# gengyuchao/SonicScribe

Measured on AMD Instinct MI355X. Metric: 20s-segments/sec/node + RTF, GLM-ASR-Nano bf16, batch=32, 1/2/4/8 MI355X, higher is better.
Workload: dtype bf16

## Files before the change

### sonicscribe_amd/csrc/attn.hip

```cpp
#include "common.h"
#include "kernels.h"
#include "int8_util.h"
#include <type_traits>


typedef unsigned u32x2_t __attribute__((ext_vector_type(2)));
__device__ __forceinline__ float rows_sum(float v) {
    u32x2_t a = __builtin_amdgcn_permlane16_swap(__float_as_uint(v), __float_as_uint(v), false, false);
    const float s = __uint_as_float(a[0]) + __uint_as_float(a[1]);
    u32x2_t b = __builtin_amdgcn_permlane32_swap(__float_as_uint(s), __float_as_uint(s), false, false);
    return __uint_as_float(b[0]) + __uint_as_float(b[1]);
}
__device__ __forceinline__ float rows_max(float v) {
    u32x2_t a = __builtin_amdgcn_permlane16_swap(__float_as_uint(v), __float_as_uint(v), false, false);
    const float s = fmaxf(__uint_as_float(a[0]), __uint_as_float(a[1]));
    u32x2_t b = __builtin_amdgcn_permlane32_swap(__float_as_uint(s), __float_as_uint(s), false, false);
    return fmaxf(__uint_as_float(b[0]), __uint_as_float(b[1]));
}

template <int HD> __device__ __forceinline__ int kswz(int row) {
    if (HD == 64) return ((row >> 1) & 1) | (((row >> 3) & 3) << 1);
    return ((row & 3) | (((row >> 3) & 1) << 2)) << 1;
}

// ... 274 lines not shown
    int n;
    if (a.P) {
        const int N = (a.Hq + 2 * a.Hkv) * HD;
        const int w = tid, vi = w / HALF, i = w % HALF;
        const bool act = w < (G + 2) * HALF;
        float x1 = 0.f, x2 = 0.f;
        if (act) {
            const int col = (vi < G ? (kvh * G + vi) : vi == G ? (a.Hq + kvh) : (a.Hq + a.Hkv + kvh)) * HD + i;
            if (a.dq.sca) {
                x1 = deq1(a.dq, a.P, a.ksplit, a.mpad, b, col, N); x2 = deq1(a.dq, a.P, a.ksplit, a.mpad, b, col + HALF, N);
            } else {
                float v1[8], v2[8];
#pragma unroll
                for (int ks = 0; ks < 8; ++ks) {
                    const float* p = a.P + ((long)(ks < a.ksplit ? ks : 0) * a.mpad + b) * N + col;
                    v1[ks] = p[0]; v2[ks] = p[HALF];
                }
#pragma unroll
                for (int ks = 0; ks < 8; ++ks)
                    if (ks < a.ksplit) { x1 += v1[ks]; x2 += v2[ks]; }
            }
        }
        n = min(max(a.kv_len[b], 1), a.ctx_max);
        if (act) {
            const int pos = n - 1;
            x1 = rT<T>(x1); x2 = rT<T>(x2);
            float o1 = x1, o2 = x2;
            if (vi <= G) {
                const float c = a.cs[(long)pos * HD + i], sn = a.cs[(long)pos * HD + HALF + i];
                o1 = rT<T>(rT<T>(x1 * c) + rT<T>(-x2 * sn));
                o2 = rT<T>(rT<T>(x2 * c) + rT<T>(x1 * sn));
            }
            const int row = vi < G ? vi : (vi == G ? GMAX : GMAX + 1);
            const T b1 = (T)o1, b2 = (T)o2;
            s_q[row][i] = b1; s_q[row][HALF + i] = b2;
            if (vi == G) { Kc[(long)pos * HD + i] = b1; Kc[(long)pos * HD + HALF + i] = b2; }
            if (vi == G + 1) { Vc[(long)pos * HD + i] = b1; Vc[(long)pos * HD + HALF + i] = b2; }
        }
        __syncthreads();
    } else {
        n = min(max(a.kv_len[b], 1), a.ctx_max);
    }
    KT(a, 1);
    V8 qf[4];
#pragma unroll
    for (int hs = 0; hs < 4; ++hs) {
        const V8 t = a.P ? *(const V8*)&s_q[r < G ? r : 0][hs * 32 + g * 8]
                         : *(const V8*)((const T*)a.Q + (long)b * a.Hq * HD + (kvh * G + (r < G ? r : 0)) * HD + hs * 32 + g * 8);
#pragma unroll
        for (int j = 0; j < 8; ++j) qf[hs][j] = r < G ? t[j] : (T)0.f;
    }
    float m[GMAX], lsum = 0.f, acc[GMAX][8];
#pragma unroll
    for (int h = 0; h < GMAX; ++h) {
        m[h] = -1e30f;
#pragma unroll
        for (int i = 0; i < 8; ++i) acc[h][i] = 0.f;
    }
    auto step = [&](int k0, const V8 (&kd)[4], const V8 (&vd)[4], int limit) {
        f32x4 st = {0.f, 0.f, 0.f, 0.f};
#pragma unroll
        for (int hs = 0; hs < 4; ++hs) st = ET<T>::mfma(kd[hs], qf[hs], st);
        float sc[4], mx = -1e30f;
#pragma unroll
        for (int j = 0; j < 4; ++j) { sc[j] = (k0 + g * 4 + j) < limit ? st[j] * a.scale : -1e30f; mx = fmaxf(mx, sc[j]); }
        mx = rows_max(mx);
        const float m_r = r == 0 ? m[0] : r == 1 ? m[1] : r == 2 ? m[2] : m[3];
        const float mn = fmaxf(m_r, mx);
        float ps = 0.f, pr[4];
#pragma unroll
        for (int j = 0; j < 4; ++j) { const float pv = (k0 + g * 4 + j) < limit ? __expf(sc[j] - mn) : 0.f; ps += pv; pr[j] = rT<T>(pv); }
        lsum = lsum * __expf(m_r - mn) + ps;
        if (r < 4) {
#pragma unroll
            for (int j = 0; j < 4; ++j) s_p[wid][g * 4 + j][r] = pr[j];
            if (g == 0) s_mn[wid][r] = mn;
        }
        __builtin_amdgcn_wave_barrier();
        const f32x4 mn4 = *(const f32x4*)s_mn[wid];
        f32x4 pk[4];
#pragma unroll
        for (int u = 0; u < 4; ++u) pk[u] = *(const f32x4*)s_p[wid][4 * u + g];
#pragma unroll
        for (int h = 0; h < GMAX; ++h) {
            const float alpha = __expf(m[h] - mn4[h]);
            m[h] = mn4[h];
#pragma unroll
            for (int i = 0; i < 8; ++i) {
                float t = acc[h][i] * alpha;
#pragma unroll
                for (int u = 0; u < 4; ++u) t += pk[u][h] * (float)vd[u][i];
                acc[h][i] = t;
            }
        }
        __builtin_amdgcn_wave_barrier();
    };
    const int nc = a.P ? n - 1 : n;
    for (int k0 = wid * 16; k0 < nc; k0 += NW * 16) {
        const bool more = k0 + NW * 16 < nc;
        if (more) load(k0 + NW * 16, kfn, vvn);
        step(k0, kf, vv, nc);
        if (more) {
#pragma unroll
            for (int u = 0; u < 4; ++u) { kf[u] = kfn[u]; vv[u] = vvn[u]; }
        }
    }
    if (a.P && wid == NW - 1) {
#pragma unroll
        for (int hs = 0; hs < 4; ++hs) kf[hs] = *(const V8*)&s_q[GMAX][hs * 32 + g * 8];
#pragma unroll
        for (int u = 0; u < 4; ++u) vv[u] = *(const V8*)&s_q[GMAX + 1][r * 8];
        step(0, kf, vv, 1);
    }
    KT(a, 2);
    lsum = rows_sum(lsum);
    if (g == 0 && r < 4) s_l[wid][r] = lsum;
    if (lane == 0) { s_m[wid][0] = m[0]; s_m[wid][1] = m[1]; s_m[wid][2] = m[2]; s_m[wid][3] = m[3]; }
#pragma unroll
    for (int h = 0; h < GMAX; ++h)
#pragma unroll
        for (int i = 0; i < 8; ++i) {
            const float v = rows_sum(acc[h][i]);
            if (g == 0) s_acc[wid][h][r * 8 + i] = v;
        }
    __syncthreads();
    KT(a, 3);
    for (int idx = tid; idx < G * HD; idx += 512) {
        const int h = idx / HD, e = idx % HD;
        float M = -1e30f;
#pragma unroll
        for (int w = 0; w < NW; ++w) M = fmaxf(M, s_m[w][h]);
        float num = 0.f, den = 0.f;
#pragma unroll
        for (int w = 0; w < NW; ++w) { const float f = __expf(s_m[w][h] - M); num += f * s_acc[w][h][e]; den += f * s_l[w][h]; }
        ((T*)a.O)[(long)b * a.Hq * HD + (kvh * G + h) * HD + e] = (T)(num / den);
    }
    KT(a, 4);
}
#endif

template <typename T> struct PV16;
typedef short s16x4_t __attribute__((ext_vector_type(4)));
template <> struct PV16<bf16_t> {
    static __device__ __forceinline__ f32x4 mfma(u32x2_t a, u32x2_t b, f32x4 c) {
        return __builtin_amdgcn_mfma_f32_16x16x16bf16_1k(__builtin_bit_cast(s16x4_t, a), __builtin_bit_cast(s16x4_t, b), c, 0, 0, 0);
    }
};
template <> struct PV16<f16_t> {
    static __device__ __forceinline__ f32x4 mfma(u32x2_t a, u32x2_t b, f32x4 c) {
        return __builtin_amdgcn_mfma_f32_16x16x16f16(__builtin_bit_cast(f16x4, a), __builtin_bit_cast(f16x4, b), c, 0, 0, 0);
    }
};

template <typename T, int WPE = 2>
__global__ __launch_bounds__(512, WPE) void decode_attn_kernel(DecodeAttnArgs a) {
    typedef typename ET<T>::v8 V8;
    constexpr int HD = 128, HALF = 64, GMAX = 4, NW = 8;
    __shared__ __attribute__((aligned(16))) float s_acc[NW][GMAX][HD];
    __shared__ float s_m[NW][GMAX], s_l[NW][GMAX];
    __shared__ __attribute__((aligned(16))) T s_q[GMAX + 2][HD];
    __shared__ int s_ok[OUTL_CAP];
    __shared__ float s_ox[OUTL_CAP];
    const int G = a.Hq / a.Hkv;
    const int tid = threadIdx.x, lane = tid & 63, wid = tid >> 6;
    const int r = lane & 15, g = lane >> 4;
    const int b = blockIdx.x, kvh = blockIdx.y;
    if ((int)blockIdx.y >= a.Hkv) {
        const int blk = (blockIdx.y - a.Hkv) * gridDim.x + blockIdx.x, nblk = (gridDim.y - a.Hkv) * gridDim.x;
        prefetch_share(a.pf[0], blk, nblk);
        prefetch_share(a.pf[1], blk, nblk);
        asm volatile("s_waitcnt vmcnt(0)" ::: "memory");
        return;
    }
    T* Kc = (T*)a.Kc + ((long)b * a.Hkv + kvh) * a.ctx_max * HD;
    T* Vc = (T*)a.Vc + ((long)b * a.Hkv + kvh) * a.ctx_max * HD;
    const int cm1 = a.ctx_max - 1;

    KT(a, 0);
    V8 kf[4], vv[4], kfn[4], vvn[4];
    auto load = [&](int k0, V8 (&kd)[4], V8 (&vd)[4]) {
        const int kr = min(k0 + r, cm1);
#pragma unroll
        for (int hs = 0; hs < 4; ++hs) kd[hs] = *(const V8*)(Kc + (long)kr * HD + hs * 32 + g * 8);
#pragma unroll
        for (int j = 0; j < 4; ++j) vd[j] = *(const V8*)(Vc + (long)min(k0 + 4 * g + j, cm1) * HD + r * 8);
    };
    load(wid * 16, kf, vv);

    int n;
    if (a.P && !a.dq.sca) {
        typedef typename ET<T>::v4 V4;
        const int N = (a.Hq + 2 * a.Hkv) * HD;
        const int vi = tid >> 4, i4 = (tid & 15) * 4;
        const bool act = tid < (G + 2) * 16;
        const int col = act ? (vi < G ? (kvh * G + vi) : vi == G ? (a.Hq + kvh) : (a.Hq + a.Hkv + kvh)) * HD + i4 : 0;
        f32x4 v1[8], v2[8];
        if (act) {
#pragma unroll
            for (int ks = 0; ks < 8; ++ks)
                if (ks < a.ksplit) {
                    const float* p = a.P + ((long)ks * a.mpad + b) * N + col;
                    v1[ks] = *(const f32x4*)p; v2[ks] = *(const f32x4*)(p + HALF);
                }
        }
        n = min(max(a.kv_len[b], 1), a.ctx_max);
        if (act) {
            f32x4 x1 = {0.f, 0.f, 0.f, 0.f}, x2 = {0.f, 0.f, 0.f, 0.f};
#pragma unroll
            for (int ks = 0; ks < 8; ++ks)
                if (ks < a.ksplit) {
#pragma unroll
                    for (int e = 0; e < 4; ++e) { x1[e] += v1[ks][e]; x2[e] += v2[ks][e]; }
                }
            const int pos = n - 1;
            f32x4 c = {1.f, 1.f, 1.f, 1.f}, sn = {0.f, 0.f, 0.f, 0.f};
            if (vi <= G) { c = *(const f32x4*)(a.cs + (long)pos * HD + i4); sn = *(const f32x4*)(a.cs + (long)pos * HD + HALF + i4); }
            V4 b1, b2;
#pragma unroll
            for (int e = 0; e < 4; ++e) {
                const float y1 = rT<T>(x1[e]), y2 = rT<T>(x2[e]);
                float o1 = y1, o2 = y2;
                if (vi <= G) {
                    o1 = rT<T>(rT<T>(y1 * c[e]) + rT<T>(-y2 * sn[e]));
                    o2 = rT<T>(rT<T>(y2 * c[e]) + rT<T>(y1 * sn[e]));
                }
                b1[e] = (T)o1; b2[e] = (T)o2;
            }
            const int row = vi < G ? vi : (vi == G ? GMAX : GMAX + 1);
            *(V4*)&s_q[row][i4] = b1; *(V4*)&s_q[row][HALF + i4] = b2;
            if (vi == G) { *(V4*)(Kc + (long)pos * HD + i4) = b1; *(V4*)(Kc + (long)pos * HD + HALF + i4) = b2; }
            if (vi == G + 1) { *(V4*)(Vc + (long)pos * HD + i4) = b1; *(V4*)(Vc + (long)pos * HD + HALF + i4) = b2; }
        }
        __syncthreads();
    } else if (a.P) {
        const int N = (a.Hq + 2 * a.Hkv) * HD;
        const int w = tid, vi = w / HALF, i = w % HALF;
        const bool act = w < (G + 2) * HALF;
        float x1 = 0.f, x2 = 0.f;
        const int col = act ? (vi < G ? (kvh * G + vi) : vi == G ? (a.Hq + kvh) : (a.Hq + a.Hkv + kvh)) * HD + i : 0;
        if (a.dq.sca) {
            const OutlStage os = outl_issue(a.dq, b);
            const Slab1x2 sl = slab1x2_load(a.dq, a.P, a.ksplit, a.mpad, b, col, HALF, N);
            outl_commit(a.dq, b, os, s_ok, s_ox);
            if (act) slab1x2_finish(a.dq, a.P, a.ksplit, a.mpad, b, col, HALF, N, sl, os, s_ok, s_ox, x1, x2);
        }
        if (act) {
            if (a.dq.sca) {
            } else {
                float v1[8], v2[8];
#pragma unroll
                for (int ks = 0; ks < 8; ++ks) {
                    const float* p = a.P + ((long)(ks < a.ksplit ? ks : 0) * a.mpad + b) * N + col;
                    v1[ks] = p[0]; v2[ks] = p[HALF];
                }
#pragma unroll
                for (int ks = 0; ks < 8; ++ks)
                    if (ks < a.ksplit) { x1 += v1[ks]; x2 += v2[ks]; }
            }
        }
        n = min(max(a.kv_len[b], 1), a.ctx_max);
        if (act) {
            const int pos = n - 1;
            x1 = rT<T>(x1); x2 = rT<T>(x2);
            float o1 = x1, o2 = x2;
            if (vi <= G) {
                const float c = a.cs[(long)pos * HD + i], sn = a.cs[(long)pos * HD + HALF + i];
                o1 = rT<T>(rT<T>(x1 * c) + rT<T>(-x2 * sn));
                o2 = rT<T>(rT<T>(x2 * c) + rT<T>(x1 * sn));
            }
            const int row = vi < G ? vi : (vi == G ? GMAX : GMAX + 1);
            const T b1 = (T)o1, b2 = (T)o2;
            s_q[row][i] = b1; s_q[row][HALF + i] = b2;
            if (vi == G) { Kc[(long)pos * HD + i] = b1; Kc[(long)pos * HD + HALF + i] = b2; }
            if (vi == G + 1) { Vc[(long)pos * HD + i] = b1; Vc[(long)pos * HD + HALF + i] = b2; }
        }
        __syncthreads();
    } else {
        n = min(max(a.kv_len[b], 1), a.ctx_max);
    }
    KT(a, 1);
    V8 qf[4];
#pragma unroll
    for (int hs = 0; hs < 4; ++hs) {
        const V8 t = a.P ? *(const V8*)&s_q[r < G ? r : 0][hs * 32 + g * 8]
                         : *(const V8*)((const T*)a.Q + (long)b * a.Hq * HD + (kvh * G + (r < G ? r : 0)) * HD + hs * 32 + g * 8);
#pragma unroll
        for (int j = 0; j < 8; ++j) qf[hs][j] = r < G ? t[j] : (T)0.f;
    }
    float m_r = -1e30f, lsum = 0.f;
    f32x4 acc[8];
#pragma unroll
    for (int t = 0; t < 8; ++t) acc[t] = (f32x4){0.f, 0.f, 0.f, 0.f};
    auto step = [&](int k0, const V8 (&kd)[4], const V8 (&vd)[4], int limit) {
        f32x4 st = {0.f, 0.f, 0.f, 0.f};
#pragma unroll
        for (int hs = 0; hs < 4; ++hs) st = ET<T>::mfma(kd[hs], qf[hs], st);
        float sc[4], mx = -1e30f;
#pragma unroll
        for (int j = 0; j < 4; ++j) { sc[j] = (k0 + g * 4 + j) < limit ? st[j] * a.scale : -1e30f; mx = fmaxf(mx, sc[j]); }
        mx = rows_max(mx);
        const float mn = fmaxf(m_r, mx);
        const float alpha = __expf(m_r - mn);
        m_r = mn;
        float ps = 0.f, pr[4];
#pragma unroll
        for (int j = 0; j < 4; ++j) { const float pv = ((k0 + g * 4 + j) < limit && r < G) ? __expf(sc[j] - mn) : 0.f; ps += pv; pr[j] = pv; }
        lsum = lsum * alpha + ps;
        u32x2_t pa;
        {
            typename ET<T>::v4 p4;
#pragma unroll
            for (int j = 0; j < 4; ++j) p4[j] = (T)pr[j];
            pa = __builtin_bit_cast(u32x2_t, p4);
        }
        const float a0 = __builtin_bit_cast(float, __builtin_amdgcn_readlane(__builtin_bit_cast(int, alpha), 0));
        const float a1 = __builtin_bit_cast(float, __builtin_amdgcn_readlane(__builtin_bit_cast(int, alpha), 1));
        const float a2 = __builtin_bit_cast(float, __builtin_amdgcn_readlane(__builtin_bit_cast(int, alpha), 2));
        const float a3 = __builtin_bit_cast(float, __builtin_amdgcn_readlane(__builtin_bit_cast(int, alpha), 3));
        const unsigned* w0 = (const unsigned*)&vd[0]; const unsigned* w1 = (const unsigned*)&vd[1];
        const unsigned* w2 = (const unsigned*)&vd[2]; const unsigned* w3 = (const unsigned*)&vd[3];
#pragma unroll
        for (int i = 0; i < 4; ++i) {
            u32x2_t blo, bhi;
            blo[0] = __builtin_amdgcn_perm(w1[i], w0[i], 0x05040100u); blo[1] = __builtin_amdgcn_perm(w3[i], w2[i], 0x05040100u);
            bhi[0] = __builtin_amdgcn_perm(w1[i], w0[i], 0x07060302u); bhi[1] = __builtin_amdgcn_perm(w3[i], w2[i], 0x07060302u);
            f32x4 c0 = acc[2 * i], c1 = acc[2 * i + 1];
            c0[0] *= a0; c0[1] *= a1; c0[2] *= a2; c0[3] *= a3;
            c1[0] *= a0; c1[1] *= a1; c1[2] *= a2; c1[3] *= a3;
            acc[2 * i] = PV16<T>::mfma(pa, blo, c0);
            acc[2 * i + 1] = PV16<T>::mfma(pa, bhi, c1);
        }
    };
    const int nc = a.P ? n - 1 : n;
    for (int k0 = wid * 16; k0 < nc; k0 += NW * 16) {
        const bool more = k0 + NW * 16 < nc;
        if (more) load(k0 + NW * 16, kfn, vvn);
        step(k0, kf, vv, nc);
        if (more) {
#pragma unroll
            for (int u = 0; u < 4; ++u) { kf[u] = kfn[u]; vv[u] = vvn[u]; }
        }
    }
    if (a.P && wid == NW - 1) {
#pragma unroll
        for (int hs = 0; hs < 4; ++hs) kf[hs] = *(const V8*)&s_q[GMAX][hs * 32 + g * 8];
#pragma unroll
        for (int u = 0; u < 4; ++u) vv[u] = *(const V8*)&s_q[GMAX + 1][r * 8];
        step(0, kf, vv, 1);
    }
    KT(a, 2);
    lsum = rows_sum(lsum);
    if (g == 0 && r < 4) { s_l[wid][r] = lsum; s_m[wid][r] = m_r; }
    if (g == 0) {
#pragma unroll
        for (int j = 0; j < 4; ++j) {
            *(f32x4*)&s_acc[wid][j][8 * r] = (f32x4){acc[0][j], acc[1][j], acc[2][j], acc[3][j]};
            *(f32x4*)&s_acc[wid][j][8 * r + 4] = (f32x4){acc[4][j], acc[5][j], acc[6][j], acc[7][j]};
        }
    }
    __syncthreads();
    KT(a, 3);
    float amx = 0.f;
    int nbig = 0;
    for (int idx = tid; idx < G * HD; idx += 512) {
        const int h = idx / HD, e = idx % HD;
        float M = -1e30f;
#pragma unroll
        for (int w = 0; w < NW; ++w) M = fmaxf(M, s_m[w][h]);
        float num = 0.f, den = 0.f;
#pragma unroll
        for (int w = 0; w < NW; ++w) { const float f = __expf(s_m[w][h] - M); num += f * s_acc[w][h][e]; den += f * s_l[w][h]; }
        const T ov = (T)(num / den);
        ((T*)a.O)[(long)b * a.Hq * HD + (kvh * G + h) * HD + e] = ov;
        const float av = fabsf((float)ov);
        amx = fmaxf(amx, av < LLM_INT8_THRESHOLD ? av : 0.f);
        nbig += !(av < LLM_INT8_THRESHOLD);
    }
    if (a.amax_out) {
        amx = wave_max(amx);
        const int wbig = __popcll(__ballot(nbig > 0)) > 0 ? (int)wave_sum((float)nbig) : 0;
        __syncthreads();
        if (lane == 0) { s_l[wid][0] = amx; s_m[wid][0] = (float)wbig; }
        __syncthreads();
        if (tid == 0) {
            float m = s_l[0][0], nb = s_m[0][0];
#pragma unroll
            for (int w = 1; w < NW; ++w) { m = fmaxf(m, s_l[w][0]); nb += s_m[w][0]; }
            a.amax_out[b * 4 + kvh] = m;
            if (a.big_out) a.big_out[b * 4 + kvh] = (int)nb;
        }
    }
    KT(a, 4);
}

void launch_decode_attn(const DecodeAttnArgs& a, int B, hipStream_t s) {
#ifdef SONIC_AB
    if (g_opts.decode_attn_v1) { DT_SWITCH(a.dt, T, hipLaunchKernelGGL(decode_attn_v1_kernel<T>, dim3(B, a.Hkv), dim3(512), 0, s, a)); return; }
#endif
    if (g_opts.decode_attn_occ2) { DT_SWITCH(a.dt, T, hipLaunchKernelGGL((decode_attn_kernel<T, 4>), dim3(B, a.Hkv), dim3(512), 0, s, a)); return; }
    DT_SWITCH(a.dt, T, hipLaunchKernelGGL((decode_attn_kernel<T, 2>), dim3(B, a.Hkv + (a.pf_y > 0 ? a.pf_y : 0)), dim3(512), 0, s, a));
}
```

### sonicscribe_amd/csrc/common.h

```cpp
#pragma once
#include <hip/hip_runtime.h>
#include <stdint.h>

typedef __bf16 bf16_t;
typedef __attribute__((ext_vector_type(8))) __bf16 bf16x8;
typedef __attribute__((ext_vector_type(4))) __bf16 bf16x4;
typedef __attribute__((ext_vector_type(2))) __bf16 bf16x2;
typedef __attribute__((ext_vector_type(4))) float f32x4;
typedef __attribute__((ext_vector_type(16))) float f32x16;
typedef __attribute__((ext_vector_type(4))) int i32x4;
typedef _Float16 f16_t;
typedef __attribute__((ext_vector_type(8))) _Float16 f16x8;
typedef __attribute__((ext_vector_type(4))) _Float16 f16x4;
typedef __attribute__((ext_vector_type(2))) _Float16 f16x2;

enum { DT_BF16 = 0, DT_F16 = 1, DT_F32 = 2 };
template <typename T> struct ET;
template <> struct ET<bf16_t> {
    typedef bf16x8 v8; typedef bf16x4 v4; typedef bf16x2 v2;
    static __device__ __forceinline__ f32x4 mfma(v8 a, v8 b, f32x4 c) { return __builtin_amdgcn_mfma_f32_16x16x32_bf16(a, b, c, 0, 0, 0); }
};
template <> struct ET<f16_t> {
    typedef f16x8 v8; typedef f16x4 v4; typedef f16x2 v2;
    static __device__ __forceinline__ f32x4 mfma(v8 a, v8 b, f32x4 c) { return __builtin_amdgcn_mfma_f32_16x16x32_f16(a, b, c, 0, 0, 0); }
};
typedef __attribute__((ext_vector_type(8))) float f32x8;
template <> struct ET<float> { typedef f32x8 v8; typedef f32x4 v4; };
template <typename T> __device__ __forceinline__ float rT(float x) { return (float)((T)x); }
template <> __device__ __forceinline__ float rT<f16_t>(float x) { asm volatile("" : "+v"(x)); return (float)((f16_t)x); }
#define DT_SWITCH(dt, T, ...) do { if ((dt) == DT_F16) { typedef f16_t T; __VA_ARGS__; } else { typedef bf16_t T; __VA_ARGS__; } } while (0)

#define WAVE 64

#include <mutex>
#include <set>
#include <utility>
inline void ensure_dyn_lds(const void* fn, int bytes) {
    static std::mutex mu;
    static std::set<std::pair<int, const void*>> done;
    int dev = 0;
    (void)hipGetDevice(&dev);
    std::lock_guard<std::mutex> lk(mu);
    if (done.insert({dev, fn}).second && hipFuncSetAttribute(fn, hipFuncAttributeMaxDynamicSharedMemorySize, bytes) != hipSuccess) (void)hipGetLastError();
}

struct LaunchOpts {
    int skinny_variant = 0;
    int gemm_force128 = 0;
    int no_fused_gu = 0;
    int no_fused_gu64 = 0;
    int ktrace_wave = 0;
    int gu64_split_norm = 0;
    int gu64_two_pass = 0;
    int o64_16rows = 0;
    int no_skinny48 = 0;
    int no_skinny768 = 0;
    int gemm_small_eff = 75;
    int gemm128_shallow = 0;
    int no_skinny_i8_wide = 0;
    int gemm256_stagger = 1;
    int decode_prefetch = 0;
    int decode_attn_occ2 = 0;
    int decode_attn_v1 = 0;
    int flash_variant = 2;
    int flash_enc = 1;
    int gemm256_persist = 0;
    int gemm256_persist_cus = 256;
    int gemm256_gm = 8;
};
extern thread_local LaunchOpts g_opts;

__device__ __forceinline__ float bf2f(bf16_t x) { return (float)x; }
__device__ __forceinline__ bf16_t f2bf(float x) { return (bf16_t)x; }
__device__ __forceinline__ float rbf(float x) { return (float)((bf16_t)x); }

__device__ __forceinline__ float gelu_erf(float x) {
    const float z = fabsf(x) * 0.70710678118654752440f;
    const float t = __builtin_amdgcn_rcpf(fmaf(0.3275911f, z, 1.0f));
    float p = fmaf(1.061405429f, t, -1.453152027f);
    p = fmaf(p, t, 1.421413741f);
    p = fmaf(p, t, -0.284496736f);
    p = fmaf(p, t, 0.254829592f);
    const float pe = p * t * __expf(-z * z);
    return 0.5f * x * (x >= 0.f ? 2.0f - pe : pe);
}
__device__ __forceinline__ float silu_f(float x) { return x / (1.0f + __expf(-x)); }

__device__ __forceinline__ float wave_sum(float v) {
#pragma unroll
    for (int o = 32; o > 0; o >>= 1) v += __shfl_xor(v, o, 64);
    return v;
}
__device__ __forceinline__ float wave_max(float v) {
#pragma unroll
    for (int o = 32; o > 0; o >>= 1) v = fmaxf(v, __shfl_xor(v, o, 64));
    return v;
}

struct PrefetchRange { const void* p; long bytes; };
__device__ __forceinline__ void prefetch_share(const PrefetchRange& r, int blk, int nblk) {
    if (!r.p || r.bytes <= 0) return;
    const long step = (long)blockDim.x * 16;
    const long per = ((r.bytes + nblk - 1) / nblk + step - 1) / step * step;
    const long lo = (long)blk * per, hi = lo + per < r.bytes ? lo + per : r.bytes;
    const char* q = (const char*)r.p;
    i32x4 t = {0, 0, 0, 0};
    for (long off = lo + (long)threadIdx.x * 16; off + 16 <= hi; off += step)
        asm volatile("global_load_dwordx4 %0, %1, off" : "+v"(t) : "v"(q + off) : "memory");
    asm volatile("s_waitcnt vmcnt(0)" : "+v"(t) :: "memory");
}

enum GemmEpi {
    EPI_BIAS = 0,
    EPI_BIAS_GELU = 1,
    EPI_BIAS_RESID = 2,
    EPI_SWIGLU = 3,
    EPI_QKV_VT = 4,
};

struct GemmI8 {
    const float* sca;
    const float* scb;
    const bf16_t* x16; long ldx16;
    const int* oc_cnt; const int* oc_list; int oc_ld;
    const int* row_group; int group_div;
    int row_off;
    bf16_t* defer_out; int defer_thr;
};

__host__ __device__ __forceinline__ long i8_tiled_row_off(int n, int K) { return (long)(n >> 4) * (K >> 6) * 1024 + (long)(n & 15) * 16; }
__host__ __device__ __forceinline__ long i8_tiled_k_off(int k) { return ((long)(k >> 6) << 10) + (((k >> 4) & 3) << 8) + (k & 15); }

struct GemmArgs {
    const bf16_t* A; long lda;
    const bf16_t* W;
    bf16_t* C; long ldc;
    const float* bias;
    const bf16_t* R; long ldr;
    int M, N, K;
    int batch; long strideA, strideC, strideR;
    bf16_t* Vt; int n_split; int seg_T; int vt_ld; long vt_seg_stride;
    int dt;
    GemmI8 q;
    const float* rope_cs; int rope_T, rope_ncols;
    const unsigned short* gelu_lut;
    int raster_gm;
    int w_tiled;
    int gu8;
    long long* dbg;
};
#define GELU_LUT_E0 113
#define GELU_LUT_NE 18
#define GELU_LUT_HALF (GELU_LUT_NE * 128)
#define GELU_LUT_N (2 * GELU_LUT_HALF)
__device__ __forceinline__ int gelu_lut_index(float l) {
    return (int)((__float_as_uint(l) >> 16) & 0x7FFFu) - (GELU_LUT_E0 << 7);
}
__device__ __forceinline__ int gelu_lut_slot(float l, int idx) {
    return (int)min((unsigned)idx, (unsigned)(GELU_LUT_HALF - 1)) + ((__float_as_uint(l) >> 31) ? GELU_LUT_HALF : 0);
}
__device__ __forceinline__ float gelu_lut_value(float l, int idx, unsigned t) {
    const float lo = 0.5f * l, hi = fmaxf(l, -0.0f);
    float y = __uint_as_float(t << 16);
    y = idx < 0 ? lo : y;
    y = idx >= GELU_LUT_HALF ? hi : y;
    return y;
}
bool gemm256_eligible(const GemmArgs& a, int epi);

struct KBF16 {
    typedef bf16_t elem; typedef bf16_t out; typedef bf16x8 frag; typedef f32x4 acc; static constexpr bool I8 = false;
    static __device__ __forceinline__ acc mfma(frag a, frag b, acc c) { return __builtin_amdgcn_mfma_f32_16x16x32_bf16(a, b, c, 0, 0, 0); }
};
struct KF16 {
    typedef f16_t elem; typedef f16_t out; typedef f16x8 frag; typedef f32x4 acc; static constexpr bool I8 = false;
    static __device__ __forceinline__ acc mfma(frag a, frag b, acc c) { return __builtin_amdgcn_mfma_f32_16x16x32_f16(a, b, c, 0, 0, 0); }
};
struct KI8 {
    typedef int8_t elem; typedef f16_t out; typedef i32x4 frag; typedef i32x4 acc; static constexpr bool I8 = true;
    static __device__ __forceinline__ acc mfma(frag a, frag b, acc c) { return __builtin_amdgcn_mfma_i32_16x16x64_i8(a, b, c, 0, 0, 0); }
};
#define KD_SWITCH(a, KD, ...) do { if ((a).q.sca) { typedef KI8 KD; __VA_ARGS__; } else if ((a).dt == DT_F16) { typedef KF16 KD; __VA_ARGS__; } \
                                   else { typedef KBF16 KD; __VA_ARGS__; } } while (0)
#define MB_SWITCH(mb, MB, ...) do { if ((mb) <= 1) { constexpr int MB = 1; __VA_ARGS__; } else if ((mb) == 2) { constexpr int MB = 2; __VA_ARGS__; } \
                                    else if ((mb) == 3) { constexpr int MB = 3; __VA_ARGS__; } else { constexpr int MB = 4; __VA_ARGS__; } } while (0)
#define KS8_SWITCH(K, KS8, ...) do { switch (K) { case 256: { constexpr int KS8 = 1; __VA_ARGS__; } break; case 512: { constexpr int KS8 = 2; __VA_ARGS__; } break; \
                                     case 1024: { constexpr int KS8 = 4; __VA_ARGS__; } break; default: { constexpr int KS8 = 8; __VA_ARGS__; } break; } } while (0)

struct SkinnyArgs {
    const bf16_t* X; long ldx;
    const bf16_t* W;
    float* P;
    int M, N, K, ksplit;
    int dt;
    int i8;
    const float* x_amax;
    const float* pre_P; int pre_ks, pre_mpad; const bf16_t* pre_x; bf16_t* pre_xout; const float* pre_w; float pre_eps;
    int* err;
    long long* kt;
    int kt_thread;
};
#define KT(a, slot) do { if ((a).kt && threadIdx.x == 0) { long long* kt_p_ = (a).kt; asm volatile("" : "+s"(kt_p_)); \
        const unsigned kt_i_ = __builtin_amdgcn_readfirstlane((blockIdx.y * gridDim.x + blockIdx.x) * 8u + (unsigned)(slot)); \
        kt_p_[kt_i_] = wall_clock64(); } } while (0)
#define KTW(a, slot) do { if ((a).kt && threadIdx.x == (unsigned)(a).kt_thread) { long long* kt_p_ = (a).kt; asm volatile("" : "+s"(kt_p_)); \
        const unsigned kt_i_ = __builtin_amdgcn_readfirstlane((blockIdx.y * gridDim.x + blockIdx.x) * 8u + (unsigned)(slot)); \
        kt_p_[kt_i_] = wall_clock64(); } } while (0)

void launch_gemm(const GemmArgs& a, int epi, hipStream_t s);
void launch_skinny(const SkinnyArgs& a, hipStream_t s);
int skinny_pick_ksplit(int N, int K);
bool skinny_pre_eligible(int M, int N, int K);
int skinny_pick_ksplit_i8(int N, int K);
int skinny_i8_cfg(int N, int K);
bool skinny_gu_eligible(int M, int N, int K);
void launch_skinny_gu(const SkinnyArgs& a, bf16_t* act, hipStream_t s);
// ... 6 lines not shown
```

### sonicscribe_amd/csrc/engine_options.cpp

```cpp
#include "engine_internal.h"

void drop_graphs(sonic_engine* e) { for (auto& g : e->graphs) (void)hipGraphExecDestroy(g.second); e->graphs.clear(); }
static int opt_token_logprobs(sonic_engine* e, const char*, int value) {
    const int v = value ? 1 : 0;
    if (!v && e->opt_sampling) return fail(e, SONIC_ERR_INVALID, "token_logprobs cannot be switched off while option sampling is on (its kernels are log-probability kernels)");
    if (!v && e->opt_grammar) return fail(e, SONIC_ERR_INVALID, "token_logprobs cannot be switched off while option grammar is on (its kernels are log-probability kernels)");
    if (!v && e->opt_top_logprobs) return fail(e, SONIC_ERR_INVALID, "token_logprobs cannot be switched off while option top_logprobs is on (its kernels are log-probability kernels)");
    e->opt_token_logprobs = v; drop_graphs(e);
    return v ? lp_alloc(e) : SONIC_OK;
}
static int opt_top_logprobs(sonic_engine* e, const char* key, int value) { TRY(gen_busy(e, key)); return top_enable(e, value); }
static int opt_gen(sonic_engine* e, const char* key, int value) {
    float p = e->gen_penalty; int n = e->gen_ngram; std::vector<int> sup = e->gen_suppress;
    if (!strcmp(key, "gen_repetition_penalty_milli")) p = (float)((double)value / 1000.0);
    else if (!strcmp(key, "gen_no_repeat_ngram_size")) n = value;
    else { sup.clear(); if (value >= 0) sup.push_back(value); }
    TRY(gen_busy(e, key));
    return gen_apply(e, p, n, sup.data(), (int)sup.size());
}
static int opt_sampling(sonic_engine* e, const char* key, int value) { TRY(gen_busy(e, key)); return samp_enable(e, value ? 1 : 0); }
static int opt_sampling_fill_milli(sonic_engine* e, const char* key, int value) {
    if (value != 0 && (value < 1 || value > 100000)) return fail(e, SONIC_ERR_INVALID, "sampling_fill_milli: %d is outside 0, 1 .. 100000", value);
    TRY(gen_busy(e, key)); e->opt_samp_fill_milli = value; return SONIC_OK;
}
static int opt_truncation(sonic_engine* e, const char* key, int value) { TRY(gen_busy(e, key)); return trunc_enable(e, value ? 1 : 0); }
static int opt_truncation_fill(sonic_engine* e, const char* key, int value) { TRY(gen_busy(e, key)); e->opt_trunc_fill = value ? 1 : 0; return SONIC_OK; }
static int opt_grammar(sonic_engine* e, const char* key, int value) { TRY(gen_busy(e, key)); return gram_enable(e, value ? 1 : 0); }
static int opt_request_grammar_begin(sonic_engine* e, const char*, int value) { return gram_stage_begin(e, value); }
static int opt_request_grammar(sonic_engine* e, const char*, int value) { return gram_stage_row(e, value); }
static int opt_hook_grammar_state(sonic_engine* e, const char*, int value) {
    const int b = value >> 20, st = (value & 0xfffff) - 2;
    if (value < 0 || b > 63 || e->hook_gram.empty() || st >= e->hook_gram[0]) return fail(e, SONIC_ERR_INVALID, "hook_grammar_state: row %d, state %d (arm a hook grammar first: sonic_load_tensor \"grammar.hook:<V>\")", b, st);
    e->hook_state_in[b] = st; return SONIC_OK;
}
static int opt_hook_grammar_eos(sonic_engine* e, const char*, int value) {
    if (value < 0 || e->hook_gram.empty() || e->hook_eos.size() >= 8) return fail(e, SONIC_ERR_INVALID, "hook_grammar_eos: id %d (at most 8 ids, behind an armed hook grammar)", value);
    e->hook_eos.push_back(value); return SONIC_OK;
}
static int opt_request_bias(sonic_engine* e, const char* key, int value) { TRY(gen_busy(e, key)); return bias_enable(e, value ? 1 : 0); }
static int opt_request_bias_fill(sonic_engine* e, const char* key, int value) {
    if (value < 0 || value > BIAS_MAX_ENTRIES || value > e->d.vocab) return fail(e, SONIC_ERR_INVALID, "request_bias_fill: %d is outside 0 .. %d", value, BIAS_MAX_ENTRIES);
    TRY(gen_busy(e, key)); e->opt_bias_fill = value; return SONIC_OK;
}
static int opt_forced_parallel(sonic_engine* e, const char* key, int value) {
    TRY(gen_busy(e, key));
    if (value && e->opt_draft_verify) return fail(e, SONIC_ERR_INVALID, "forced_parallel: option draft_verify is on: a scoring handle decodes nothing a draft could shorten");
    if (!value && e->opt_forced_align) return fail(e, SONIC_ERR_INVALID, "forced_parallel cannot be switched off while option forced_align is on (the alignment rides on the parallel forced run)");
    if (!value && e->opt_forced_share_prompt) return fail(e, SONIC_ERR_INVALID, "forced_parallel cannot be switched off while option forced_share_prompt is on (the shared prompt is the parallel forced run's)");
    e->opt_forced_parallel = value ? 1 : 0; return SONIC_OK;
}
static int opt_forced_share_prompt(sonic_engine* e, const char* key, int value) {
    TRY(gen_busy(e, key));
    if (value && !e->opt_forced_parallel) return fail(e, SONIC_ERR_INVALID, "forced_share_prompt: option forced_parallel must be on first (the shared prompt is the parallel forced run's; sonic_set_option(e, \"forced_parallel\", 1))");
    if (value && e->i8) return fail(e, SONIC_ERR_INVALID, "forced_share_prompt: not on an int8 handle (its prefill finds outlier columns per sequence - one sequence = one reference call - and a shared prompt belongs to several)");
    if (value && e->f32) return fail(e, SONIC_ERR_INVALID, "forced_share_prompt: the fp32 kind has no shared-prefix attention kernel; use a bf16 or fp16 handle");
    if (value && e->opt_forced_align) return fail(e, SONIC_ERR_INVALID, "forced_share_prompt: option forced_align is on (the alignment kernels read a sequence's audio keys from its own row)");
    e->opt_forced_share_prompt = value ? 1 : 0; return SONIC_OK;
}
static int opt_forced_fanout(sonic_engine* e, const char* key, int value) {
    if (value < 1 || value > e->Bm) return fail(e, SONIC_ERR_INVALID, "forced_fanout: %d is outside 1 .. %d (max_batch)", value, e->Bm);
    e->opt_forced_fanout = value; return SONIC_OK;
}
static int opt_draft_verify(sonic_engine* e, const char* key, int value) { TRY(gen_busy(e, key)); return draft_enable(e, value ? 1 : 0); }
static int opt_forced_align(sonic_engine* e, const char* key, int value) {
    TRY(gen_busy(e, key));
    if (value && e->f32) return fail(e, SONIC_ERR_INVALID, "forced_align: the fp32 kind has no alignment kernels (its prefill keeps no roped queries); use a bf16 or int8-mode handle");
    if (value && e->opt_forced_share_prompt) return fail(e, SONIC_ERR_INVALID, "forced_align: option forced_share_prompt is on (the alignment kernels read a sequence's audio keys from its own row); switch it off first");
    if (value && !e->opt_forced_parallel) return fail(e, SONIC_ERR_INVALID, "forced_align: option forced_parallel must be on first (the alignment rides on the parallel forced run; sonic_set_option(e, \"forced_parallel\", 1))");
    e->opt_forced_align = value ? 1 : 0;
    if (!value) e->align_last = false;
    return SONIC_OK;
}
static int opt_align_head(sonic_engine* e, const char* key, int value) {
    TRY(gen_busy(e, key));
    if (value == -1) { e->align_heads.clear(); return SONIC_OK; }
    const int l = value >> 8, h = value & 255;
    if (value < 0 || l >= e->d.dec_layers || h >= e->d.dec_heads) return fail(e, SONIC_ERR_INVALID, "align_head: %d (layer %d, head %d) is outside %d layers x %d heads", value, l, h, e->d.dec_layers, e->d.dec_heads);
    if (std::find(e->align_heads.begin(), e->align_heads.end(), value) != e->align_heads.end()) return SONIC_OK;
    if (e->align_heads.size() >= ALIGN_MAX_HEADS) return fail(e, SONIC_ERR_INVALID, "align_head: the list already holds %d heads", ALIGN_MAX_HEADS);
    e->align_heads.insert(std::upper_bound(e->align_heads.begin(), e->align_heads.end(), value), value);
    return SONIC_OK;
}
static int opt_ktrace(sonic_engine* e, const char*, int value) {
    HIPC(e, hipSetDevice(e->device));
    if (value >= 0 && !e->kt) { TRY(dalloc(e, &e->kt, (size_t)8 * KT_SLOT_BLOCKS * 8)); }
    if (e->kt) zero_fill(e, e->kt, (size_t)8 * KT_SLOT_BLOCKS * 8 * 8);
    e->kt_layer = value; drop_graphs(e); return SONIC_OK;
}
static int opt_inject_dev_err(sonic_engine* e, const char*, int value) {
    HIPC(e, hipSetDevice(e->device));
    const int v = value ? 1 : 0;
    HIPC(e, hipMemcpyAsync(e->n_active + 1, &v, 4, hipMemcpyHostToDevice, e->st));
    HIPC(e, stream_sync(e));
    return SONIC_OK;
}

struct OptRow { const char* key; int sonic_engine::* field; int LaunchOpts::* lfield; bool drop_graphs; int (*clamp)(int); int (*apply)(sonic_engine*, const char* key, int value); };
#define ENG(m) &sonic_engine::m, nullptr
#define LOP(m) nullptr, &LaunchOpts::m
#define APPLY(f) nullptr, nullptr, false, nullptr, f
static const OptRow OPTIONS[] = {
    {"skinny_variant", LOP(skinny_variant), true, nullptr},
    {"gemm_force128", LOP(gemm_force128), false, nullptr},
    {"no_fused_gu", LOP(no_fused_gu), true, nullptr},
    {"no_fused_gu64", LOP(no_fused_gu64), true, nullptr},
    {"gu64_two_pass", LOP(gu64_two_pass), true, nullptr},
    {"gu64_split_norm", LOP(gu64_split_norm), true, nullptr},
    {"ktrace_wave", LOP(ktrace_wave), true, nullptr},
    {"no_skinny768", LOP(no_skinny768), true, nullptr},
    {"no_skinny48", LOP(no_skinny48), true, nullptr},
    {"o64_16rows", LOP(o64_16rows), true, nullptr},
    {"i8_no_lnq", ENG(opt_i8_no_lnq), false, nullptr},
    {"i8_no_qkv_fuse", ENG(opt_i8_no_qkv_fuse), false, nullptr},
    {"i8_dbg", ENG(opt_i8_dbg), true, nullptr},
    {"i8_no_xq", ENG(opt_i8_no_xq), true, nullptr},
    {"gemm_small_eff", LOP(gemm_small_eff), false, nullptr},
    {"gemm128_shallow", LOP(gemm128_shallow), false, nullptr},
    {"no_skinny_i8_wide", LOP(no_skinny_i8_wide), true, nullptr},
    {"gemm256_stagger", LOP(gemm256_stagger), false, nullptr},
    {"flash_variant", LOP(flash_variant), false, nullptr},
    {"flash_enc", LOP(flash_enc), false, nullptr},
    {"gemm256_persist", LOP(gemm256_persist), false, nullptr},
    {"gemm256_persist_cus", LOP(gemm256_persist_cus), false, [](int v) { return v > 0 ? v : 256; }},
    {"gemm256_gm", LOP(gemm256_gm), false, [](int v) { return v > 0 ? v : 8; }},
    {"i8_defer_thr", ENG(opt_i8_defer_thr), false, nullptr},
    {"decode_prefetch", LOP(decode_prefetch), true, nullptr},
    {"decode_attn_occ2", LOP(decode_attn_occ2), true, nullptr},
    {"decode_attn_v1", LOP(decode_attn_v1), true, nullptr},
    {"prefill_taps", ENG(taps_on), false, nullptr},
    {"no_pre_norm", ENG(opt_no_pre_norm), true, nullptr},
    {"decode_gemv", ENG(opt_decode_gemv), true, nullptr},
    {"f32_synth_bf16", ENG(opt_f32_synth_bf16), false, nullptr},
    {"no_graph", ENG(opt_no_graph), false, nullptr},
    {"decode_lookahead", ENG(lookahead), false, [](int v) { return v < 1 ? 1 : (v > CHK_MAX_AHEAD ? CHK_MAX_AHEAD : v); }},
    {"decode_chunk", ENG(opt_decode_chunk), false, [](int v) { return v > 0 ? (v > 64 ? 64 : v) : 1; }},
    {"prefill_rowmajor", ENG(opt_prefill_rowmajor), false, nullptr},
    {"no_rope_tiles", ENG(opt_no_rope_tiles), false, nullptr},
    {"gemm_trace", ENG(opt_gemm_trace), false, nullptr},
    {"gemm_timing", ENG(opt_gemm_timing), false, nullptr},
    {"no_fused_rope", ENG(opt_no_fused_rope), false, nullptr},
    {"no_gelu_lut", ENG(opt_no_gelu_lut), false, nullptr},
    {"token_logprobs", APPLY(opt_token_logprobs)},
    {"top_logprobs", APPLY(opt_top_logprobs)},
    {"gen_repetition_penalty_milli", APPLY(opt_gen)},
    {"gen_no_repeat_ngram_size", APPLY(opt_gen)},
    {"gen_suppress_token", APPLY(opt_gen)},
    {"sampling", APPLY(opt_sampling)},
    {"sampling_fill_milli", APPLY(opt_sampling_fill_milli)},
    {"truncation", APPLY(opt_truncation)},
    {"truncation_fill", APPLY(opt_truncation_fill)},
    {"grammar", APPLY(opt_grammar)},
    {"request_grammar_begin", APPLY(opt_request_grammar_begin)},
    {"request_grammar", APPLY(opt_request_grammar)},
    {"hook_grammar_state", APPLY(opt_hook_grammar_state)},
    {"hook_grammar_eos", APPLY(opt_hook_grammar_eos)},
    {"request_bias", APPLY(opt_request_bias)},
    {"request_bias_fill", APPLY(opt_request_bias_fill)},
    {"forced_parallel", APPLY(opt_forced_parallel)},
    {"forced_fanout", APPLY(opt_forced_fanout)},
    {"forced_share_prompt", APPLY(opt_forced_share_prompt)},
    {"forced_align", APPLY(opt_forced_align)},
    {"align_head", APPLY(opt_align_head)},
    {"draft_verify", APPLY(opt_draft_verify)},
    {"score_chunk_rows", ENG(opt_score_chunk_rows), false, [](int v) { return v < 16 ? 16 : (v > 4096 ? 4096 : v); }},
    {"ktrace", APPLY(opt_ktrace)},
    {"inject_dev_err", APPLY(opt_inject_dev_err)},
};
extern "C" int sonic_set_option(sonic_engine* e, const char* key, int value) {
    if (!e || !key) return SONIC_ERR_INVALID;
    if (!strncmp(key, "request_grammar", 15)) {
        std::lock_guard<std::mutex> ak(e->a_mu);
        if (e->a_pending || e->a_running) return fail(nullptr, SONIC_ERR_INVALID, "%s: an asynchronous run of this handle is in flight", key);
    }
    std::lock_guard<std::mutex> lk(e->mu);
    for (const OptRow& r : OPTIONS) {
        if (strcmp(key, r.key)) continue;
        if (r.apply) return r.apply(e, key, value);
        const int v = r.clamp ? r.clamp(value) : value;
        if (r.field) e->*r.field = v; else e->opts.*r.lfield = v;
        if (r.drop_graphs) drop_graphs(e);
        return SONIC_OK;
    }
    return fail(e, SONIC_ERR_INVALID, "unknown option %s", key);
}

struct DbgRow { const char* name; size_t (*cap)(const sonic_engine*); const bf16_t* (*src16)(const sonic_engine*); const float* (*src32)(const sonic_engine*);
                const float* (*f32_on_16)(const sonic_engine*) = nullptr;
                int (*n_idx)(const sonic_engine*) = nullptr; };
#define CAP(x) [](const sonic_engine* e) -> size_t { return x; }
#define S16(m) [](const sonic_engine* e) -> const bf16_t* { return e->m; }
#define S32(m) [](const sonic_engine* e) -> const float* { return e->f->m; }
static const DbgRow DEBUG_BUFS[] = {
    {"prefill_tap", CAP((size_t)e->tok_cap * e->d.dec_d), S16(taps), [](const sonic_engine* e) -> const float* { return (const float*)e->taps; }, nullptr, [](const sonic_engine* e) -> int { return e->d.dec_layers + 1; }},
    {"kcache", CAP((size_t)e->Bm * e->d.dec_kv_heads * e->max_ctx * e->d.dec_head_dim), S16(Kc), nullptr, nullptr, [](const sonic_engine* e) -> int { return e->d.dec_layers; }},
    {"vcache", CAP((size_t)e->Bm * e->d.dec_kv_heads * e->max_ctx * e->d.dec_head_dim), S16(Vc), nullptr, nullptr, [](const sonic_engine* e) -> int { return e->d.dec_layers; }},
    {"pe", CAP((size_t)e->Bm * e->Ta * e->d.dec_d), S16(pe), S32(pe)},
    {"dx", CAP((size_t)e->tok_cap * e->d.dec_d), S16(dx), S32(dx)},
    {"dqkv", CAP((size_t)e->tok_cap * e->qkvN), S16(dqkv), nullptr},
    {"dq", CAP((size_t)e->tok_cap * e->QD), S16(dq), nullptr},
    {"datt", CAP((size_t)e->tok_cap * e->QD), S16(datt), nullptr},
    {"dact", CAP((size_t)e->tok_cap * e->d.dec_ff), S16(dact), nullptr},
    {"enc_x", CAP((size_t)e->Bm * e->T * e->d.enc_d), S16(ln), S32(ln)},
    {"h1", CAP((size_t)e->Bm * (e->d.n_frames + 2) * e->d.enc_d), nullptr, S32(h1)},
    {"shn", CAP((size_t)64 * e->d.dec_d), S16(shn), nullptr},
    {"satt", CAP((size_t)64 * e->QD), S16(satt), nullptr},
    {"sact", CAP((size_t)64 * e->d.dec_ff), S16(sact), nullptr},
    {"align_probs", CAP(e->align_P ? (size_t)e->align_last_heads * e->align_S * e->align_Amax : 0), nullptr, nullptr, [](const sonic_engine* e) -> const float* { return e->align_P; }},
    {"align_matrix", CAP(e->align_M ? (size_t)e->align_S * e->align_Amax : 0), nullptr, nullptr, [](const sonic_engine* e) -> const float* { return e->align_M; }},
};
extern "C" int sonic_debug_read(sonic_engine* e, const char* name, int index, float* out, int64_t n) {
    if (!e || !name || !out) return SONIC_ERR_INVALID;
    ENTER(e);
    if (!strcmp(name, "hook_grammar_state")) {
        if (n < 0 || n > 64) return fail(e, SONIC_ERR_INVALID, "read of %lld elements exceeds buffer %s", (long long)n, name);
        for (int64_t i = 0; i < n; ++i) out[i] = (float)e->hook_state_out[i];
        return SONIC_OK;
    }
    if (!strcmp(name, "hook_truncation")) {
        if (n < 0 || n > 64 * 3) return fail(e, SONIC_ERR_INVALID, "read of %lld elements exceeds buffer %s", (long long)n, name);
        for (int64_t i = 0; i < n; ++i) { if (i % 3 == 0) memcpy(&out[i], &e->hook_trunc_rec[i], 4); else out[i] = (float)(int)e->hook_trunc_rec[i]; }
        return SONIC_OK;
    }
    if (!strcmp(name, "draft_accepted")) {
        if (n < 0 || n > 64) return fail(e, SONIC_ERR_INVALID, "read of %lld elements exceeds buffer %s", (long long)n, name);
        if (!e->opt_draft_verify) return fail(e, SONIC_ERR_INVALID, "draft_accepted: option draft_verify is off on this handle");
        int acc[64] = {0};
        if (e->draft_last_S > 0 && e->draft_acc) { HIPC(e, stream_sync(e)); HIPC(e, d2h(e, acc, e->draft_acc, 64 * 4)); }
        for (int64_t i = 0; i < n; ++i) out[i] = (float)acc[i];
        return SONIC_OK;
    }
    if (!strcmp(name, "score_tokens")) {
        if (n != 1) return fail(e, SONIC_ERR_INVALID, "read of %lld elements exceeds buffer %s", (long long)n, name);
        out[0] = (float)e->score_tokens;
        return SONIC_OK;
    }
    if (!strcmp(name, "fork_ms")) {
        if (n != 1) return fail(e, SONIC_ERR_INVALID, "read of %lld elements exceeds buffer %s", (long long)n, name);
        out[0] = 0.f;
        if (e->fork_timed) { HIPC(e, stream_sync(e)); HIPC(e, hipEventElapsedTime(&out[0], e->fork_ev[0], e->fork_ev[1])); }
        return SONIC_OK;
    }
    for (const DbgRow& r : DEBUG_BUFS) {
        if (strcmp(name, r.name) || !(e->f32 ? (bool)r.src32 : (r.src16 || r.f32_on_16))) continue;
        const bool tap = &r == &DEBUG_BUFS[0];
        if (tap && !e->taps) return fail(e, SONIC_ERR_INVALID, "no taps recorded");
        if (r.n_idx && (index < 0 || index >= r.n_idx(e))) return fail(e, SONIC_ERR_INVALID, "index %d out of range for buffer %s (0 .. %d)", index, name, r.n_idx(e) - 1);
        const size_t cap = r.cap(e), off = r.n_idx ? (size_t)index * cap : 0;
        if (n < 0 || (size_t)n > cap) return fail(e, SONIC_ERR_INVALID, "read of %lld elements exceeds buffer %s", (long long)n, name);
        if (!e->f32 && r.f32_on_16) { HIPC(e, stream_sync(e)); if (n > 0) HIPC(e, d2h(e, out, r.f32_on_16(e), (size_t)n * 4)); return SONIC_OK; }
        if (!e->f32) return read_back_16(e, r.src16(e) + off, out, (size_t)n);
        HIPC(e, stream_sync(e)); HIPC(e, d2h(e, out, r.src32(e) + off, (size_t)n * 4));
        return SONIC_OK;
    }
    return fail(e, SONIC_ERR_INVALID, "unknown buffer %s", name);
}

extern "C" int sonic_debug_ktrace(sonic_engine* e, int64_t* out, int64_t n) {
    if (!e || !out) return SONIC_ERR_INVALID;
    ENTER(e);
    if (!e->kt) return fail(e, SONIC_ERR_INVALID, "ktrace is off");
    const int64_t have = (int64_t)8 * KT_SLOT_BLOCKS * 8;
    HIPC(e, stream_sync(e));
    HIPC(e, d2h(e, out, e->kt, (size_t)(n < have ? n : have) * 8));
    return SONIC_OK;
}
```

Before: 172.2.

## Reorder decode attention loads to overlap KV fetch with QKV reduction and RoPE

Adds a new default decode-attention variant that issues the first two K/V tiles, kv_len, the split-K partial sums and the RoPE cos/sin loads through inline asm with explicit vmcnt waits. The split-K reduction and RoPE run while later KV tiles are still in flight, and the first two loop iterations are peeled. The aim is to hide global-memory latency at kernel start, where the K/V loads used to wait behind the QKV epilogue. In exchange it relies on hand-counted vmcnt values that must match the number of outstanding loads, which is fragile, and it keeps the old path behind an option.

```diff
diff --git a/sonicscribe_amd/csrc/attn.hip b/sonicscribe_amd/csrc/attn.hip
--- a/sonicscribe_amd/csrc/attn.hip
+++ b/sonicscribe_amd/csrc/attn.hip
@@ -450,17 +450,34 @@
     }
 };
 
-template <typename T, int WPE = 2>
+template <int N> __device__ __forceinline__ void da_wait_vm() { asm volatile("s_waitcnt vmcnt(%0)" ::"n"(N) : "memory"); }
+__device__ __forceinline__ void da_wait_kvlen(int slabs) {
+    switch (slabs) {
+        case 0: da_wait_vm<8>(); break;
+        case 1: da_wait_vm<10>(); break;
+        case 2: da_wait_vm<12>(); break;
+        case 3: da_wait_vm<14>(); break;
+        case 4: da_wait_vm<16>(); break;
+        case 5: da_wait_vm<18>(); break;
+        case 6: da_wait_vm<20>(); break;
+        case 7: da_wait_vm<22>(); break;
+        case 8: da_wait_vm<24>(); break;
+        default: da_wait_vm<0>(); break;
+    }
+}
+template <typename T, int WPE = 2, int ORD = 1>
 __global__ __launch_bounds__(512, WPE) void decode_attn_kernel(DecodeAttnArgs a) {
     typedef typename ET<T>::v8 V8;
     constexpr int HD = 128, HALF = 64, GMAX = 4, NW = 8;
+    static_assert(ORD == 1 || WPE == 2, "the new issue order is built for the 2-waves-per-SIMD allocation");
     __shared__ __attribute__((aligned(16))) float s_acc[NW][GMAX][HD];
     __shared__ float s_m[NW][GMAX], s_l[NW][GMAX];
     __shared__ __attribute__((aligned(16))) T s_q[GMAX + 2][HD];
     __shared__ int s_ok[OUTL_CAP];
     __shared__ float s_ox[OUTL_CAP];
     const int G = a.Hq / a.Hkv;
-    const int tid = threadIdx.x, lane = tid & 63, wid = tid >> 6;
+    const int tid = threadIdx.x, lane = tid & 63;
+    const int wid = ORD == 0 ? __builtin_amdgcn_readfirstlane(tid >> 6) : tid >> 6;
     const int r = lane & 15, g = lane >> 4;
     const int b = blockIdx.x, kvh = blockIdx.y;
     if ((int)blockIdx.y >= a.Hkv) {
@@ -483,10 +500,91 @@
 #pragma unroll
         for (int j = 0; j < 4; ++j) vd[j] = *(const V8*)(Vc + (long)min(k0 + 4 * g + j, cm1) * HD + r * 8);
     };
-    load(wid * 16, kf, vv);
+    auto issue = [&](int k0, V8 (&kd)[4], V8 (&vd)[4]) {
+        const T* kp = Kc + (long)min(k0 + r, cm1) * HD + g * 8;
+#pragma unroll
+        for (int hs = 0; hs < 4; ++hs) asm volatile("global_load_dwordx4 %0, %1, off offset:%2" : "=v"(kd[hs]) : "v"(kp), "n"(hs * 32 * (int)sizeof(T)) : "memory");
+#pragma unroll
+        for (int j = 0; j < 4; ++j) asm volatile("global_load_dwordx4 %0, %1, off" : "=v"(vd[j]) : "v"(Vc + (long)min(k0 + 4 * g + j, cm1) * HD + r * 8) : "memory");
+    };
+    auto landed = [&](V8 (&kd)[4], V8 (&vd)[4]) {
+#pragma unroll
+        for (int u = 0; u < 4; ++u) asm volatile("" : "+v"(kd[u]), "+v"(vd[u]));
+    };
+    int nraw = 0;
+    if constexpr (ORD == 0) {
+        asm volatile("global_load_dword %0, %1, off" : "=v"(nraw) : "v"(a.kv_len + b) : "memory");
+        issue(wid * 16, kf, vv);
+    } else {
+        load(wid * 16, kf, vv);
+    }
 
     int n;
-    if (a.P && !a.dq.sca) {
+    if constexpr (ORD == 0) {
+        typedef typename ET<T>::v4 V4;
+        const int N = (a.Hq + 2 * a.Hkv) * HD;
+        const int vi = tid >> 4, i4 = (tid & 15) * 4;
+        const bool act = tid < (G + 2) * 16;
+        const bool wact = a.P && wid * 64 < (G + 2) * 16;
+        const int col = act ? (vi < G ? (kvh * G + vi) : vi == G ? (a.Hq + kvh) : (a.Hq + a.Hkv + kvh)) * HD + i4 : 0;
+        const int nslab = wact ? min(max(a.ksplit, 0), 8) : 0;
+        f32x4 v1[8], v2[8], c, sn;
+        if (wact) {
+#pragma unroll
+            for (int ks = 0; ks < 8; ++ks)
+                if (ks < nslab) {
+                    const float* p = a.P + ((long)ks * a.mpad + b) * N + col;
+                    asm volatile("global_load_dwordx4 %0, %1, off" : "=v"(v1[ks]) : "v"(p) : "memory");
+                    asm volatile("global_load_dwordx4 %0, %1, off offset:256" : "=v"(v2[ks]) : "v"(p) : "memory");
+                }
+        }
+        da_wait_kvlen(nslab);
+        asm volatile("" : "+v"(nraw));
+        n = min(max(__builtin_amdgcn_readfirstlane(nraw), 1), a.ctx_max);
+        const int pos = n - 1;
+        if (wact) {
+            const float* cp = a.cs + (long)pos * HD + i4;
+            asm volatile("global_load_dwordx4 %0, %1, off" : "=v"(c) : "v"(cp) : "memory");
+            asm volatile("global_load_dwordx4 %0, %1, off offset:256" : "=v"(sn) : "v"(cp) : "memory");
+        }
+        issue(wid * 16 + NW * 16, kfn, vvn);
+        if (wact) {
+            da_wait_vm<8>();
+            asm volatile("" : "+v"(c), "+v"(sn));
+#pragma unroll
+            for (int ks = 0; ks < 8; ++ks)
+                if (ks < nslab) asm volatile("" : "+v"(v1[ks]), "+v"(v2[ks]));
+            if (act) {
+                f32x4 x1 = {0.f, 0.f, 0.f, 0.f}, x2 = {0.f, 0.f, 0.f, 0.f};
+#pragma unroll
+                for (int ks = 0; ks < 8; ++ks)
+                    if (ks < nslab) {
+#pragma unroll
+                        for (int e = 0; e < 4; ++e) { x1[e] += v1[ks][e]; x2[e] += v2[ks][e]; }
+                    }
+                V4 b1, b2;
+#pragma unroll
+                for (int e = 0; e < 4; ++e) {
+                    const float y1 = rT<T>(x1[e]), y2 = rT<T>(x2[e]);
+                    float o1 = y1, o2 = y2;
+                    if (vi <= G) {
+                        o1 = rT<T>(rT<T>(y1 * c[e]) + rT<T>(-y2 * sn[e]));
+                        o2 = rT<T>(rT<T>(y2 * c[e]) + rT<T>(y1 * sn[e]));
+                    }
+                    b1[e] = (T)o1; b2[e] = (T)o2;
+                }
+                const int row = vi < G ? vi : (vi == G ? GMAX : GMAX + 1);
+                *(V4*)&s_q[row][i4] = b1; *(V4*)&s_q[row][HALF + i4] = b2;
+                if (vi == G) { *(V4*)(Kc + (long)pos * HD + i4) = b1; *(V4*)(Kc + (long)pos * HD + HALF + i4) = b2; }
+                if (vi == G + 1) { *(V4*)(Vc + (long)pos * HD + i4) = b1; *(V4*)(Vc + (long)pos * HD + HALF + i4) = b2; }
+            }
+        }
+        if (a.P) {
+            asm volatile("s_waitcnt lgkmcnt(0)" ::: "memory");
+            __builtin_amdgcn_s_barrier();
+            asm volatile("" ::: "memory");
+        }
+    } else if (a.P && !a.dq.sca) {
         typedef typename ET<T>::v4 V4;
         const int N = (a.Hq + 2 * a.Hkv) * HD;
         const int vi = tid >> 4, i4 = (tid & 15) * 4;
@@ -580,10 +678,30 @@
     V8 qf[4];
 #pragma unroll
     for (int hs = 0; hs < 4; ++hs) {
+        if constexpr (ORD == 0) continue;
         const V8 t = a.P ? *(const V8*)&s_q[r < G ? r : 0][hs * 32 + g * 8]
                          : *(const V8*)((const T*)a.Q + (long)b * a.Hq * HD + (kvh * G + (r < G ? r : 0)) * HD + hs * 32 + g * 8);
 #pragma unroll
         for (int j = 0; j < 8; ++j) qf[hs][j] = r < G ? t[j] : (T)0.f;
+    }
+    if constexpr (ORD == 0) {
+        if (a.P) {
+#pragma unroll
+            for (int hs = 0; hs < 4; ++hs) {
+                const V8 t = *(const V8*)&s_q[r < G ? r : 0][hs * 32 + g * 8];
+#pragma unroll
+                for (int j = 0; j < 8; ++j) qf[hs][j] = r < G ? t[j] : (T)0.f;
+                asm volatile("" : "+v"(qf[hs]));
+            }
+        } else {
+#pragma unroll
+            for (int hs = 0; hs < 4; ++hs) {
+                const V8 t = *(const V8*)((const T*)a.Q + (long)b * a.Hq * HD + (kvh * G + (r < G ? r : 0)) * HD + hs * 32 + g * 8);
+#pragma unroll
+                for (int j = 0; j < 8; ++j) qf[hs][j] = r < G ? t[j] : (T)0.f;
+                asm volatile("" : "+v"(qf[hs]));
+            }
+        }
     }
     float m_r = -1e30f, lsum = 0.f;
     f32x4 acc[8];
@@ -630,13 +748,37 @@
         }
     };
     const int nc = a.P ? n - 1 : n;
-    for (int k0 = wid * 16; k0 < nc; k0 += NW * 16) {
-        const bool more = k0 + NW * 16 < nc;
-        if (more) load(k0 + NW * 16, kfn, vvn);
-        step(k0, kf, vv, nc);
-        if (more) {
-#pragma unroll
-            for (int u = 0; u < 4; ++u) { kf[u] = kfn[u]; vv[u] = vvn[u]; }
+    if constexpr (ORD == 0) {
+        int k0 = wid * 16;
+        da_wait_vm<8>();
+        landed(kf, vv);
+        bool s3 = false;
+        if (k0 < nc) {
+            step(k0, kf, vv, nc);
+            s3 = k0 + 2 * NW * 16 < nc;
+            if (s3) load(k0 + 2 * NW * 16, kf, vv);
+        }
+        if (s3) da_wait_vm<8>(); else da_wait_vm<0>();
+        landed(kfn, vvn);
+        if (k0 + NW * 16 < nc) step(k0 + NW * 16, kfn, vvn, nc);
+        for (k0 += 2 * NW * 16; k0 < nc; k0 += NW * 16) {
+            const bool more = k0 + NW * 16 < nc;
+            if (more) load(k0 + NW * 16, kfn, vvn);
+            step(k0, kf, vv, nc);
+            if (more) {
+#pragma unroll
+                for (int u = 0; u < 4; ++u) { kf[u] = kfn[u]; vv[u] = vvn[u]; }
+            }
+        }
+    } else {
+        for (int k0 = wid * 16; k0 < nc; k0 += NW * 16) {
+            const bool more = k0 + NW * 16 < nc;
+            if (more) load(k0 + NW * 16, kfn, vvn);
+            step(k0, kf, vv, nc);
+            if (more) {
+#pragma unroll
+                for (int u = 0; u < 4; ++u) { kf[u] = kfn[u]; vv[u] = vvn[u]; }
+            }
         }
     }
     if (a.P && wid == NW - 1) {
@@ -696,5 +838,9 @@
     if (g_opts.decode_attn_v1) { DT_SWITCH(a.dt, T, hipLaunchKernelGGL(decode_attn_v1_kernel<T>, dim3(B, a.Hkv), dim3(512), 0, s, a)); return; }
 #endif
     if (g_opts.decode_attn_occ2) { DT_SWITCH(a.dt, T, hipLaunchKernelGGL((decode_attn_kernel<T, 4>), dim3(B, a.Hkv), dim3(512), 0, s, a)); return; }
+    if (!g_opts.decode_attn_order && !a.dq.sca) {
+        DT_SWITCH(a.dt, T, hipLaunchKernelGGL((decode_attn_kernel<T, 2, 0>), dim3(B, a.Hkv + (a.pf_y > 0 ? a.pf_y : 0)), dim3(512), 0, s, a));
+        return;
+    }
     DT_SWITCH(a.dt, T, hipLaunchKernelGGL((decode_attn_kernel<T, 2>), dim3(B, a.Hkv + (a.pf_y > 0 ? a.pf_y : 0)), dim3(512), 0, s, a));
 }
diff --git a/sonicscribe_amd/csrc/common.h b/sonicscribe_amd/csrc/common.h
--- a/sonicscribe_amd/csrc/common.h
+++ b/sonicscribe_amd/csrc/common.h
@@ -62,6 +62,7 @@
     int decode_prefetch = 0;
     int decode_attn_occ2 = 0;
     int decode_attn_v1 = 0;
+    int decode_attn_order = 0;
     int flash_variant = 2;
     int flash_enc = 1;
     int gemm256_persist = 0;
diff --git a/sonicscribe_amd/csrc/engine_options.cpp b/sonicscribe_amd/csrc/engine_options.cpp
--- a/sonicscribe_amd/csrc/engine_options.cpp
+++ b/sonicscribe_amd/csrc/engine_options.cpp
@@ -127,6 +127,7 @@
     {"decode_prefetch", LOP(decode_prefetch), true, nullptr},
     {"decode_attn_occ2", LOP(decode_attn_occ2), true, nullptr},
     {"decode_attn_v1", LOP(decode_attn_v1), true, nullptr},
+    {"decode_attn_order", LOP(decode_attn_order), true, nullptr},
     {"prefill_taps", ENG(taps_on), false, nullptr},
     {"no_pre_norm", ENG(opt_no_pre_norm), true, nullptr},
     {"decode_gemv", ENG(opt_decode_gemv), true, nullptr},
```

Result: no change. 170.9 (-0.7%).
